# rasmusab/bayes.js

Measured on AMD Instinct MI355X. Metric: posterior draws/sec (= param-updates/sec), higher is better.
Workload: dtype f64

## Files before the change

bayes.js_amd/csrc/amwg_eval.h:

```cpp
#pragma once
#include "amwg_kernel.h"
#include "amwg_user.h"

namespace amwg {

AMWG_HD double ld_by_id(int id, double x, double a, double b, double c) {
  switch (id) {
    case 0: return ld_norm(x, a, b);
    case 1: return ld_unif(x, a, b);
    case 2: return ld_beta(x, a, b);
    case 3: return ld_bern(x, a);
    case 4: return ld_pois(x, a);
    case 5: return ld_cauchy(x, a, b);
    case 6: return ld_laplace(x, a, b);
    case 7: return ld_gamma(x, a, b);
    case 8: return ld_invgamma(x, a, b);
    case 9: return ld_lnorm(x, a, b);
    case 10: return ld_pareto(x, a, b);
    case 11: return ld_t(x, a, b, c);
    case 12: return ld_weibull(x, a, b);
    case 13: return ld_logis(x, a, b);
    case 14: return ld_exp(x, a);
    case 15: return ld_binom(x, a, b);
    case 16: return ld_nbinom(x, a, b);
// ... 61 lines not shown
    case 19: r = quot_plain(x, y); break;
    case 20: r = math1_by_id((int)y, x); break;
    case 21: r = atan2_v8(x, y); break;
    case 22: r = hypot3_v8(x, y, z); break;
    case 23: r = hypot2_v8(x, y); break;
    case 24: r = js_mod(x, y); break;
    case 25: r = (double)js_toint32(x); break;
    case 26: { double lam; r = exp_log_v8(x, lam, exp_log_regs()); } break;
    case 27: { double lam; (void)exp_log_v8(x, lam, exp_log_regs()); r = lam; } break;
    case 28: r = exp_v8_full(x); break;
    case 29: r = log_v8_full(x); break;
    case 30: r = log_v8_full(exp_v8_full(x)); break;
    case 31: { double lam; r = exp_log_v8(x, lam, ExpLogLiterals{}); } break;
    case 32: r = log1p_exp_v8(x); break;
    case 33: r = log1p_exp_v8(x, exp_log_regs()); break;
    case 34: r = log1p_v8(exp_v8_full(x)); break;
    case 35: { bool rare = false; r = log1p_exp_v8_open(rare, x); if (rare) r = log1p_exp_cold(x); } break;
    case 36: r = softplus_bounded(x); break;
    case 37: r = softplus_bounded(x, softplus_regs()); break;
  }
  out[i] = r;
}

}
```

bayes.js_amd/csrc/amwg_kernel.h:

```cpp
#pragma once
#if !defined(__HIPCC_RTC__)
#include <hip/hip_runtime.h>
#endif

#include "amwg_div.h"
#include "amwg_ld.h"
#include "amwg_philox.h"
#include "amwg_types.h"

namespace amwg {

struct LdsLayout {
  uint32_t data, state, pls, cnt, tot, cc, adapt, pl, idx, perm, total, stride, logpls, bc, xw;
};
__host__ __device__ inline LdsLayout lds_layout(size_t data_bytes, int P, int CPB, int max_top, int n_named, bool multi = false) {
  LdsLayout L;
  uint32_t o = 0;
  L.stride = (uint32_t)P | 1u;
  L.data = o;  o += (uint32_t)((data_bytes + 15) & ~(size_t)15);
  L.state = o; o += L.stride * CPB * 8;
  L.pls = o;   o += L.stride * CPB * 8;
  L.cnt = o;   o += L.stride * CPB * 8;
  L.tot = o;   o += (L.stride * CPB * 4 + 15) & ~15u;
  L.cc = o;    o += (uint32_t)P * sizeof(CompConst);
  L.adapt = o; o += ((uint32_t)P + 7) & ~7u;
  L.pl = o;    o += (uint32_t)n_named * 20u;
  o = (o + 15) & ~15u;
  L.idx = o;   o += (max_top > 1) ? (((uint32_t)max_top * CPB * (max_top > kByteTop ? 2u : 1u) + 15) & ~15u) : 0;
  L.perm = o;  o += (n_named > kPackedNamed) ? (((uint32_t)n_named * CPB * 2u + 15) & ~15u) : 0;
  L.logpls = o; o += multi ? L.stride * CPB * 8 : 0;
// ... 213 lines not shown
    b0 = consumed >> 1;
    pos = (uint32_t)(consumed & 1u);
    fill();
  }
  __device__ __forceinline__ uint64_t consumed() const { return 2 * b0 + (uint64_t)pos; }
  __device__ __forceinline__ double next() {
    if constexpr (L == 64) {
      uint32_t p = (uint32_t)__builtin_amdgcn_readfirstlane((int)pos);
      if (p >= 128u) { b0 += 64ull; p = 0u; fill(); }
      const double mine = (p & 1u) ? u1 : u0;
      const int src = (int)(p >> 1);
      const uint32_t hi = (uint32_t)__builtin_amdgcn_readlane((int)(f64_bits(mine) >> 32), src);
      const uint32_t lo = (uint32_t)__builtin_amdgcn_readlane((int)(uint32_t)f64_bits(mine), src);
      pos = p + 1u;
      return bits_f64(((uint64_t)hi << 32) | (uint64_t)lo);
    } else {
      if (pos >= 2u * (uint32_t)L) { b0 += (uint64_t)L; pos = 0u; fill(); }
      double mine = (pos & 1u) ? u1 : u0;
      if constexpr (L > 1) mine = __shfl(mine, base_lane + (int)(pos >> 1), 64);
      ++pos;
      return mine;
    }
  }
};

template <int G>
__device__ __forceinline__ bool chain_true(bool c) {
#if defined(__HIP_DEVICE_COMPILE__)
  if constexpr (G >= 64) return __ballot(c) != 0ull;
#endif
  return c;
}

__device__ inline __attribute__((noinline)) int certified_test_wide(double dA, double eta, double u) {
  const double lo = dA - eta, hi = dA + eta;
  if (hi < -746.0) return -1;
  if (lo >= 0.0) return 1;
  if (!(eta < 0x1p+9) || !(u > 0x1p-60)) return 0;
  if (exp_v8(lo) * (1.0 - 0x1p-50) > u) return 1;
  if (exp_v8(hi) * (1.0 + 0x1p-50) < u) return -1;
  return 0;
}
__device__ __forceinline__ int certified_test(double dA, double eta, double ex, double u) {
  if (eta < 0x1p-7) return (ex * (1.0 - eta) > u && (u > 0.0 || dA > -700.0)) ? 1 : (ex * (1.0 + eta) < u ? -1 : 0);
  return certified_test_wide(dA, eta, u);
}

template <class Rng>
__device__ __forceinline__ double rnorm_js(Rng &rng, double mean, double sd) {
  constexpr int GU = Rng::kLanesPerChain;
  double u, v, q;
  bool again;
  do {
    u = rng.next();
    v = 1.7156 * (rng.next() - 0.5);
    const double x = u - 0.449871;
    const double y = __builtin_fabs(v) + 0.386595;
    q = x * x + y * (0.19600 * y - 0.25472 * x);
    again = false;
    if (chain_true<GU>(q > 0.27597)) again = chain_true<GU>(q > 0.27846) || chain_true<GU>(v * v > -4 * log_v8_cold(u) * u * u);
  } while (again);
  return (v / u) * sd + mean;
}

struct IndexColumn {
  unsigned char *base;
  int CPB;
  bool wide;
  __device__ __forceinline__ int get(int t) const {
    return wide ? (int)reinterpret_cast<const uint16_t *>(base)[t * CPB] : (int)base[t * CPB];
  }
  __device__ __forceinline__ void set(int t, int v) const {
    if (wide) reinterpret_cast<uint16_t *>(base)[t * CPB] = (uint16_t)v; else base[t * CPB] = (uint8_t)v;
  }
};
__device__ __forceinline__ uint32_t perm_get(uint64_t perm, int i) { return (uint32_t)(perm >> (4 * i)) & 0xFu; }
__device__ __forceinline__ uint64_t perm_swap(uint64_t perm, int i, int j) {
  const uint64_t d = ((perm >> (4 * i)) ^ (perm >> (4 * j))) & 0xFull;
  return perm ^ (d << (4 * i)) ^ (d << (4 * j));
}

__device__ __forceinline__ double js_max2(double a, double b) {
  if (a != a || b != b) return __builtin_nan("");
  if (a == b) return (a == 0 && __builtin_signbit(a)) ? b : a;
  return a > b ? a : b;
}

template <class M, int G, bool GL, bool SW = false> struct RngOf { using type = CoopStream<G>; };
template <class M, int G> struct RngOf<M, G, true, false> { using type = typename M::Stream; };
template <class M, int G> struct RngOf<M, G, false, true> { using type = typename M::SweepStream; };
template <class M, class = void> struct DynamicLdsOf { static constexpr bool value = false; };
template <class M> struct DynamicLdsOf<M, void_of<decltype(M::kDynamicLds)>> { static constexpr bool value = M::kDynamicLds; };
template <class M, bool GL> struct DataBytesOf {
  static __device__ __forceinline__ size_t get(const DataRef &d, int lanes, int threads) {
    if constexpr (DynamicLdsOf<M>::value) return M::lds_bytes_of(d, lanes, threads);
    else return M::lds_bytes(d.n_obs, d.G, lanes);
  }
};
template <class M> struct DataBytesOf<M, true> { static __device__ __forceinline__ size_t get(const DataRef &d, int, int threads) { return M::gl_lds_bytes(d.pad, threads / 64); } };

#if defined(__HIP_DEVICE_COMPILE__)
typedef const StepArgs __attribute__((address_space(4))) *cold_args_ptr;
__device__ __forceinline__ cold_args_ptr cold_args() {
  cold_args_ptr p = (cold_args_ptr)__builtin_amdgcn_kernarg_segment_ptr();
  asm volatile("" : "+s"(p));
  return p;
}
#else
typedef const StepArgs *cold_args_ptr;
__device__ inline cold_args_ptr cold_args() { return nullptr; }
#endif

struct SlotPre {
// ... 75 lines not shown
#endif
  return v;
}

__device__ __forceinline__ double lane_value(double v, int src) {
#if defined(__HIP_DEVICE_COMPILE__)
  const uint32_t hi = (uint32_t)__builtin_amdgcn_readlane((int)(f64_bits(v) >> 32), src);
  const uint32_t lo = (uint32_t)__builtin_amdgcn_readlane((int)(uint32_t)f64_bits(v), src);
  return bits_f64(((uint64_t)hi << 32) | (uint64_t)lo);
#else
  return v;
#endif
}

constexpr int kErrReplicasNeedOneWave = 1, kErrLaunchTooLong = 2, kErrMirrorOutOfSync = 4, kErrSweepNeedsOrderInRegisters = 8, kErrNoKernelBody = 16;
__device__ __forceinline__ void device_error(const StepArgs &a, int code) {
#if defined(__HIP_DEVICE_COMPILE__)
  if (threadIdx.x == 0) (void)atomicOr(a.ch.error, code);
#endif
}
template <class M, class = void> struct MirrorCheckOf { static constexpr bool value = false; };
template <class M> struct MirrorCheckOf<M, void_of<decltype(M::kMirrorCheck)>> { static constexpr bool value = M::kMirrorCheck; };

template <class Model, int G, int BT = 256, bool GL = false, bool SW = false, bool CT = false>
__device__ __forceinline__ void step_body(const StepArgs &a, unsigned char *smem) {
  constexpr int kPassU = SW ? (CertNeedsRows<Model>::value ? 2 : 4) : (BT >= 1024 ? 4 : 8);
  const int tid = threadIdx.x, nt = blockDim.x;
  constexpr bool kMulti = G > 64;
  if (!kMulti && a.cpb > 0 && nt != 64) { device_error(a, kErrReplicasNeedOneWave); return; }
  if (a.n_steps > 65535) { device_error(a, kErrLaunchTooLong); return; }
  const int CPB = kMulti ? G / 64 : ((a.cpb > 0 && a.cpb < nt / G) ? a.cpb : nt / G);
  const int c_raw = kMulti ? tid / 64 : tid / G;
  const int c_in = c_raw < CPB ? c_raw : CPB - 1, sub = tid % G;
  const int P = a.pl.P;
  const int n_named = a.pl.n_params;
  const LdsLayout L = lds_layout(DataBytesOf<Model, GL>::get(a.d, G, nt), P, CPB, a.pl.max_top, n_named, kMulti);

  const unsigned char *data_lds = smem + L.data;
  double *Sblk = reinterpret_cast<double *>(smem + L.state);
  CompConst *cc = reinterpret_cast<CompConst *>(smem + L.cc);
  uint8_t *adapt = smem + L.adapt;
  int32_t *pl_base = reinterpret_cast<int32_t *>(smem + L.pl), *pl_len = pl_base + n_named, *pl_top = pl_len + n_named, *pl_multidim = pl_top + n_named, *pl_inner = pl_multidim + n_named;
  const bool wide_idx = a.pl.max_top > kByteTop, wide_perm = n_named > kPackedNamed;
  const IndexColumn idx{smem + L.idx + (wide_idx ? 2 * c_in : c_in), CPB, wide_idx};
  const IndexColumn pcol{smem + L.perm + 2 * c_in, CPB, true};
  double *SDme = reinterpret_cast<double *>(smem + L.pls) + (size_t)c_in * L.stride;
  int2 *CNTme = reinterpret_cast<int2 *>(smem + L.cnt) + (size_t)c_in * L.stride;
// ... 7 lines not shown
  for (int p = tid; p < P; p += nt) { cc[p] = a.cc[p]; adapt[p] = a.is_adapting[p]; }
  for (int i = tid; i < 4 * n_named; i += nt) pl_base[i] = a.pl.tab[i];
  for (int i = tid; i < n_named; i += nt) pl_inner[i] = a.pl.tab[n_named + i] / a.pl.tab[2 * n_named + i];

  const int64_t chain_raw = kMulti ? (int64_t)blockIdx.x : (int64_t)blockIdx.x * CPB + c_in;
  const bool live = chain_raw < a.C;
  const int64_t cl = live ? chain_raw : a.C - 1;
  const bool writer = live && sub == 0;
  const bool counter = sub == 0 && c_raw < CPB;
  const int64_t C = a.C;

  double *Sme = Sblk + (size_t)c_in * L.stride;
  for (int p = 0; p < P; ++p) {
    Sme[p] = a.ch.state[p * C + cl];
    SDme[p] = exp_v8(a.ch.prop_log_scale[p * C + cl]);
    CNTme[p] = make_int2(a.ch.acceptance_count[p * C + cl], a.ch.iterations_since_adaption[p * C + cl]);
    TOTme[p] = 0u;
    if constexpr (kMulti) { LOGPLSme[p] = a.ch.prop_log_scale[p * C + cl]; BCme[p] = a.ch.batch_count[p * C + cl]; }
  }
  const StateView S{Sme};
  uint64_t perm = wide_perm ? 0ull : a.ch.perm[cl];
  if (wide_perm)
    for (int k = 0; k < n_named; ++k) pcol.set(k, (int)a.ch.perm16[(int64_t)k * C + cl]);
  typename RngOf<Model, G, GL, SW>::type rng;
  if constexpr (GL) rng.init(a.seed, a.chain_offset + (uint64_t)cl, a.ch.rng_n[cl], tid, reinterpret_cast<double *>(smem + L.data + Model::gl_lds_bytes(a.d.pad, 0)) + (size_t)(tid >> 6) * 256);
  else if constexpr (SW) rng.init(a.seed, a.chain_offset + (uint64_t)cl, a.ch.rng_n[cl], tid, reinterpret_cast<double *>(smem + L.data + Model::window_offset(a.d, nt / 64)) + (size_t)(tid >> 6) * 256);
  else rng.init(a.seed, a.chain_offset + (uint64_t)cl, a.ch.rng_n[cl], tid);
  double lp_curr = a.ch.lp_curr[cl];
  __syncthreads();
  constexpr bool kCert = CT && CertifiedAt<Model, G>::value && !GL && (SW == CertNeedsRows<Model>::value);
  static_assert(kCert == CT, "a certified kernel is instantiated for a model that has no certified value at this lane count");
  constexpr bool kRefOrder = kCert && G > 1 && RefOrderOf<Model>::value;
  auto expression = [&]() -> double {
    if constexpr (kRefOrder) return Model::template reference_order<G>(cache, S, a.mc, a.d, data_lds, sub);
    else if constexpr (!GL) return log_post<Model, G, kPassU>(S, a, data_lds, sub, xw, cache);
    else return 0.0;
  };
  if constexpr (!GL) { if (a.init_lp) lp_curr = expression(); }
  double lpA = lp_curr, epsA = 0.0;
  bool lp_exact = true;
  if constexpr (kCert) { if (!a.init_lp) { epsA = a.ch.lp_eps[cl]; lp_exact = epsA == 0.0; } }
  (void)lpA; (void)epsA; (void)lp_exact;
#if defined(AMWG_AUDIT)
  constexpr bool kAudit = kCert;
#else
  constexpr bool kAudit = false;
#endif
  [[maybe_unused]] double audE = 0.0, aud_max_v = 0.0, aud_max_d = 0.0;
  [[maybe_unused]] uint32_t aud_n = 0u, aud_bad = 0u;
// ... 268 lines not shown
          p_s = p;
          rng.pos = p;
          if (t_begin < top) p_s = rng.position();
        }
        lp_curr = Model::total(gl, lane64, gl.pm, gl.pt, gl.T);
      }
    }
  } else
  for (int step = 0; step < n_steps; ++step) {
    AMWG_PHASE(15);
    record_draws(step);
    shuffle_named();
    AMWG_PHASE(0);
    int np = 0, e = 0, e_top = 0, e_in = 0;
    double sw_prop = 0.0, sw_u = 0.0;
    int ord_pos = lane64;
    (void)ord_pos;
    int sw_left = 0;
    int sb = 0;
    if constexpr (kSweep) sb = Model::sweep_base(a.d);
    bool sw_pending = false;
    int d_len = 1, d_base = 0, d_multi = 0, d_inner = 1;
    auto next_comp = [&]() -> int {
      if (e == 0) {
        const int p = chain_uniform<G>(wide_perm ? pcol.get(np) : (int)perm_get(perm, np));
        d_len = chain_uniform<G>(pl_len[p]);
        d_base = chain_uniform<G>(pl_base[p]);
        d_multi = chain_uniform<G>(pl_multidim[p]);
        if (d_multi) {
          const int top = chain_uniform<G>(pl_top[p]);
          d_inner = chain_uniform<G>(pl_inner[p]);
          if (ord_in_regs) {
#if defined(__HIP_DEVICE_COMPILE__)
            if constexpr (kSweep) {
              const uint32_t p0 = rng.position();
              rng.ensure_b();
              const double uf = rng.at(lane64 >= 1 && lane64 < top ? p0 + (uint32_t)(top - 1 - lane64) : 0u);
              const int jv = (int)__builtin_floor(uf * (double)(lane64 + 1));
              int posc = lane64, i = top - 1;
              for (; i >= 4; i -= 4) {
                const int j0 = __builtin_amdgcn_readlane(jv, i), j1 = __builtin_amdgcn_readlane(jv, i - 1), j2 = __builtin_amdgcn_readlane(jv, i - 2), j3 = __builtin_amdgcn_readlane(jv, i - 3);
                posc = posc == i ? j0 : (posc == j0 ? i : posc);
                posc = posc == i - 1 ? j1 : (posc == j1 ? i - 1 : posc);
                posc = posc == i - 2 ? j2 : (posc == j2 ? i - 2 : posc);
                posc = posc == i - 3 ? j3 : (posc == j3 ? i - 3 : posc);
              }
              for (; i > 0; --i) {
                const int j = __builtin_amdgcn_readlane(jv, i);
                posc = posc == i ? j : (posc == j ? i : posc);
              }
              rng.pos = p0 + (uint32_t)(top - 1);
              ord_pos = posc;
              ord = __builtin_amdgcn_ds_permute(posc << 2, lane64);
            } else if constexpr (G >= 64) {
              ord = lane64;
              for (int i = top - 1; i > 0; --i) {
                const int j = __builtin_amdgcn_readfirstlane((int)__builtin_floor(rng.next() * (double)(i + 1)));
                const int ti = __builtin_amdgcn_readlane(ord, i), tj = __builtin_amdgcn_readlane(ord, j);
                ord = lane64 == i ? tj : (lane64 == j ? ti : ord);
              }
            }
#endif
          } else {
            for (int t = 0; t < top; ++t) idx.set(t, t);
            for (int i = top - 1; i > 0; --i) {
              const int j = (int)__builtin_floor(rng.next() * (double)(i + 1));
              const int ti = idx.get(i);
              idx.set(i, idx.get(j));
              idx.set(j, ti);
            }
          }
          if constexpr (kSweep) sw_pending = sweep_rt && d_base == Model::sweep_base(a.d) && d_inner == 1 && d_len == chain_uniform<G>(Model::sweep_len(a.d)) && d_len > 1;
        }
      }
      int comp = d_base;
      if (d_multi) {
        int t = 0;
        if (ord_in_regs) {
#if defined(__HIP_DEVICE_COMPILE__)
          if constexpr (G >= 64) t = __builtin_amdgcn_readlane(ord, __builtin_amdgcn_readfirstlane(e_top));
#endif
        } else t = idx.get(e_top);
        comp += t * d_inner + e_in;
        if (++e_in == d_inner) { e_in = 0; ++e_top; }
      }
      if (++e == d_len) { e = 0; e_top = 0; e_in = 0; ++np; }
      return comp;
    };
    auto prefetch = [&](int comp) -> SlotPre {
      SlotPre q;
      q.comp = comp;
      q.cur = Sme[comp];
      q.sd = SDme[comp];
      q.cnt = CNTme[comp];
      q.batch_size = cc[comp].batch_size;
// ... 216 lines not shown
        set_state(comp, 1.0);
        const double one_ld = log_post<Model, G, kPassU>(S, a, data_lds, sub, xw, cache);
        const double mx = js_max2(zero_ld, one_ld);
        const double z = zero_ld - mx, o = one_ld - mx;
        const double zero_prob = exp_v8(z - log_v8(exp_v8(z) + exp_v8(o)));
        double now = 1.0;
        lp_curr = one_ld;
        if (rng.next() < zero_prob) { set_state(comp, 0.0); now = 0.0; lp_curr = zero_ld; }
        if (counter) (void)__hip_atomic_fetch_add(&TOTme[comp], 1u + ((now != old) ? 0x10000u : 0u), __ATOMIC_RELAXED, __HIP_MEMORY_SCOPE_WORKGROUP);
        if (slot + 1 < P_stepped) nx = prefetch(next_comp());
        continue;
      }
      AMWG_PHASE(14);
      const double cur = me.cur;
      const bool in_sweep = kSweep && sw_left > 0;
      double prop;
      if (in_sweep) prop = lane_value(sw_prop, comp - sb);
      else {
        prop = rnorm_js(rng, cur, me.sd);
        if (chain_true<G>(k_type == kTypeInt)) prop = js_round(prop);
      }
      const bool inb = chain_true<G>(!(prop < k_lower || prop > k_upper));
      double u_accept = 0.0;
      if (inb) { set_state(comp, prop); u_accept = in_sweep ? lane_value(sw_u, comp - sb) : rng.next(); }
      if (in_sweep) --sw_left;
      AMWG_PHASE(8);
      if (slot + 1 < P_stepped) nx = prefetch(next_comp());
      AMWG_PHASE(9);
      bool accepted = false;
      bool certified = false;
      [[maybe_unused]] double aud_E_prop = 0.0;
      if constexpr (kCert) {
        if (__ballot(inb) != 0ull) {
          wave_priority(0);
          const typename Model::Approx r = Model::template log_post_approx<G, BT>(cache, S, a.mc, a.d, data_lds, sub);
          wave_priority(kStepperPriority);
          AMWG_PHASE(10);
          if (inb) {
            const double dA = r.value - lpA;
            const double eta = ((r.eps + epsA + __builtin_fabs(dA) * 0x1p-51) * 1.0625 + 0x1p-49) * a.bound_scale;
            const double ex = exp_v8(dA);
            if constexpr (kAudit) { if (a.audit_adversarial) u_accept = audit_adversarial_u(ex, eta, u_accept, step + slot); }
            const int verdict = certified_test(dA, eta, ex, u_accept);
            if constexpr (kAudit) {
              aud_E_prop = expression();
              audit_value(r.value, r.eps, aud_E_prop);
              audit_difference(dA, (r.eps + epsA + __builtin_fabs(dA) * 0x1p-51) * 1.0625, aud_E_prop - audE, verdict, u_accept);
// ... 121 lines not shown
```

bayes.js_amd/csrc/amwg_plan.hip:

```cpp
#include <algorithm>
#include <cmath>
#include <cstdlib>

#include "amwg_host.h"
#include "amwg_kernel.h"
#include "amwg_models.h"

using namespace amwg;

const FamilyRow *family_of(int model) {
  static const FamilyRow rows[4] = {amwg_family_row<0>(), amwg_family_row<1>(), amwg_family_row<2>(), amwg_family_row<3>()};
  return model >= AMWG_MODEL_NORMAL && model <= AMWG_MODEL_POIS_GLM ? &rows[model - 1] : nullptr;
}

int gl_layout(const double *y, const int32_t *g, int N, int Gn, GlLayoutHost *out) {
  if (Gn < 1 || Gn > 64) return amwg_fail(AMWG_EINVAL, "group_local: 1 to 64 groups (a chain runs on one wavefront, a lane serves one group), got %d", Gn);
  std::vector<int> n(Gn, 0), L(Gn, 1), first(Gn, 0);
  for (int i = 0; i < N; ++i) {
    if (g[i] < 0 || g[i] >= Gn) return amwg_fail(AMWG_EINVAL, "group_local: g[%d] = %d outside 0..%d", i, g[i], Gn - 1);
    n[g[i]]++;
  }
  int total = Gn;
  for (;;) {
    int best = 0;
// ... 72 lines not shown
  const bool cert = decide_certified && ((s->model == AMWG_MODEL_NORMAL && G == 1) || (s->model == AMWG_MODEL_POIS_GLM && G == 16) || rows) &&
                    family_of(s->model)->certified(G, bt).plain != nullptr;
  p.variant = rows ? (cert ? Variant::HierSweepCert : Variant::HierSweep) : (cert ? Variant::StepCert : Variant::Step);
  p.pad = rows ? HierNormalModel::row_pitch(s->d.n_obs) : ((cert && s->model == AMWG_MODEL_NORMAL && bt <= 512 && !o.sufficient_statistics) ? 1 : 0);
  return p;
}

static bool row_layout(const amwg_sampler *s, const LaunchPlan &p) {
  return p.variant == Variant::HierSweep || p.variant == Variant::HierSweepCert || (s->user && p.pad > 0);
}

static uint32_t lds_of_size(const amwg_sampler *s, const LaunchPlan &p, int cpb, int n_obs) {
  const int G = p.lanes, bt = p.block;
  size_t data = 0;
  switch (p.variant) {
    case Variant::GroupLocal: data = HierGlModel::gl_lds_bytes(p.pad, bt / 64); break;
    case Variant::HierSweep: case Variant::HierSweepCert: data = HierNormalModel::rows_lds_bytes(p.pad, bt / 64, s->d.G); break;
    case Variant::Step: case Variant::StepCert:
      data = (s->model == AMWG_MODEL_NORMAL && G == 1) ? (p.pad ? NormalModel::one_lane_tile_bytes(n_obs) : 0) : family_of(s->model)->lds_bytes(n_obs, s->d.G, G);
      break;
    default:
      data = p.pad ? HierNormalModel::rows_lds_bytes(p.pad, bt / 64, s->user_rows_groups) : (size_t)(G == 1 ? s->user_lds_one_lane : s->user_lds);
  }
  return G > 64 ? lds_layout(data, s->P, G / 64, s->pl.max_top, s->n_params, true).total : lds_layout(data, s->P, cpb ? cpb : bt / G, s->pl.max_top, s->n_params).total;
}

static uint32_t lds_of(const amwg_sampler *s, const LaunchPlan &p, int cpb = 0) {
  if (s->n_datasets <= 1) return lds_of_size(s, p, cpb, s->d.n_obs);
  uint32_t most = 0;
  int last = -1;
  for (int n : s->ds_n_obs) {
    if (n == last) continue;
    most = std::max(most, lds_of_size(s, p, cpb, n));
    last = n;
  }
  return most;
}

static int priced_n_obs(const amwg_sampler *s) {
  if (s->n_datasets <= 1) return s->d.n_obs;
  int64_t sum = 0;
  for (int n : s->ds_n_obs) sum += n;
  return (int)((sum + s->n_datasets - 1) / s->n_datasets);
}
static int log2_of(int lanes) { int lg = 0; for (int g = lanes; g > 1; g >>= 1) ++lg; return lg; }
static double model_work(const amwg_sampler *s, int G) {
  const LaunchPlan q = variant_for(s, G, 256, (size_t)160 * 1024);
// ... 228 lines not shown
```

bayes.js_amd/csrc/amwg_rtc.hip:

```cpp
#include <hip/hiprtc.h>
#include <fcntl.h>
#include <sys/stat.h>
#include <unistd.h>

#include <cstdio>
#include <cstdlib>
#include <cstring>
#include <map>
#include <mutex>

#include "amwg_host.h"

extern "C" {
extern const char amwg_hdr_stdint[], amwg_hdr_types[], amwg_hdr_math[], amwg_hdr_div[], amwg_hdr_ld[], amwg_hdr_philox[],
    amwg_hdr_kernel[], amwg_hdr_user[], amwg_hdr_twoval[], amwg_hdr_kval[], amwg_hdr_trig[], amwg_hdr_pass[], amwg_hdr_rows[], amwg_hdr_window[], amwg_hdr_gtail[],
    amwg_hdr_user_kernels[], amwg_hdr_user_dataset[];
}

static std::string user_program(const char *source, int lanes, int block) {
  return "#include \"amwg_kernel.h\"\n#include \"amwg_user.h\"\n#define AMWG_USER_LANES " + std::to_string(lanes) + "\n#define AMWG_USER_BLOCK " + std::to_string(block) + "\n" +
         source + "\n#include \"amwg_user_kernels.h\"\n";
}

namespace {
struct CacheKey { uint64_t h1, h2, h3; uint64_t len; };
CacheKey hash_key(const std::vector<std::string> &parts) {
  CacheKey k{0xcbf29ce484222325ull, 0x84222325cbf29ce4ull, 0x9e3779b97f4a7c15ull, 0};
  for (const std::string &p : parts) {
    for (unsigned char c : p) {
      k.h1 = (k.h1 ^ c) * 0x100000001b3ull;
      k.h2 = (k.h2 + c + (k.h2 << 6) + (k.h2 >> 2)) * 0xff51afd7ed558ccdull;
      k.h3 = ((k.h3 << 5) | (k.h3 >> 59)) ^ (c * 0xc4ceb9fe1a85ec53ull);
    }
    k.h1 = (k.h1 ^ 0xff) * 0x100000001b3ull;
    k.len += p.size() + 1;
  }
  return k;
}
// ... 38 lines not shown
void cache_write(const std::string &dir, const std::string &file, const CacheKey &k, const std::vector<char> &code) {
  make_dirs(dir);
  if (!cache_dir_trusted(dir)) return;
  const std::string tmp = file + ".tmp." + std::to_string((long)getpid());
  const int fd = open(tmp.c_str(), O_WRONLY | O_CREAT | O_EXCL | O_NOFOLLOW | O_CLOEXEC, 0600);
  if (fd < 0) return;
  FILE *f = fdopen(fd, "wb");
  if (!f) { close(fd); (void)remove(tmp.c_str()); return; }
  const uint64_t hdr[4] = {k.h2, k.h3, k.len, payload_sum(code)}, n = code.size();
  const bool ok = fwrite(kCacheMagic, 1, 8, f) == 8 && fwrite(hdr, 8, 4, f) == 4 && fwrite(&n, 8, 1, f) == 1 && fwrite(code.data(), 1, code.size(), f) == code.size();
  if (fclose(f) != 0 || !ok || rename(tmp.c_str(), file.c_str()) != 0) (void)remove(tmp.c_str());
}
std::atomic<int> g_cache_hits{0}, g_cache_misses{0};
}

static void dump_code_object(const std::vector<char> &code) {
  if (const char *dump = getenv("AMWG_DUMP_CODE_OBJECT")) {
    if (FILE *f = fopen(dump, "wb")) { fwrite(code.data(), 1, code.size(), f); fclose(f); }
  }
}

static int compile_user(const char *source, int lanes, int block, const char *arch, std::vector<char> *code, bool datasets, bool use_cache = true) {
  static const char *names[] = {"amwg_stdint.h", "amwg_types.h", "amwg_math.h", "amwg_div.h", "amwg_ld.h", "amwg_philox.h", "amwg_kernel.h", "amwg_user.h",
                                "amwg_twoval.h", "amwg_kval.h", "amwg_trig.h", "amwg_pass.h", "amwg_rows.h", "amwg_window.h", "amwg_gtail.h", "amwg_user_kernels.h", "amwg_user_dataset.h"};
  const char *texts[] = {amwg_hdr_stdint, amwg_hdr_types, amwg_hdr_math, amwg_hdr_div, amwg_hdr_ld, amwg_hdr_philox, amwg_hdr_kernel, amwg_hdr_user,
                         amwg_hdr_twoval, amwg_hdr_kval, amwg_hdr_trig, amwg_hdr_pass, amwg_hdr_rows, amwg_hdr_window, amwg_hdr_gtail, amwg_hdr_user_kernels, amwg_hdr_user_dataset};
  constexpr int kHeaders = (int)(sizeof(texts) / sizeof(texts[0]));
  const std::string prog_src = user_program(source, lanes, block);
#if defined(AMWG_AUDIT)
  const char *const kOpts[] = {"-O3", "-std=c++17", "-ffp-contract=off", "-fno-fast-math", "-Wno-unused-value", "-DAMWG_AUDIT=1"};
#elif defined(AMWG_X_PHASES)
  const char *const kOpts[] = {"-O3", "-std=c++17", "-ffp-contract=off", "-fno-fast-math", "-Wno-unused-value", "-DAMWG_X_PHASES=1"};
#else
  const char *const kOpts[] = {"-O3", "-std=c++17", "-ffp-contract=off", "-fno-fast-math", "-Wno-unused-value", "-falign-loops=64"};
#endif
  static const char *const kDatasetsOpt = "-DAMWG_USER_DATASETS=1";
  std::string dir = cache_dir(), file;
  CacheKey key{};
  if (!dir.empty()) {
    int rt_major = 0, rt_minor = 0;
    (void)hiprtcVersion(&rt_major, &rt_minor);
    std::vector<std::string> parts = {prog_src, arch, "hiprtc " + std::to_string(rt_major) + "." + std::to_string(rt_minor)};
    for (const char *o : kOpts) parts.push_back(o);
    if (datasets) parts.push_back(kDatasetsOpt);
    for (const char *t : texts) parts.push_back(t);
    key = hash_key(parts);
    char name[64];
    snprintf(name, sizeof name, "/%016llx%016llx.hsaco", (unsigned long long)key.h1, (unsigned long long)key.h2);
    file = dir + name;
// ... 100 lines not shown
```

bayes.js_amd/csrc/amwg_rtc_headers.c:

```c
#define AMWG_TEXT(sym, file)                                                        \
  __asm__(".section .rodata\n.global " #sym "\n.type " #sym ", @object\n" #sym ":\n" \
          ".incbin \"" file "\"\n.byte 0\n.size " #sym ", .-" #sym "\n.text\n")
AMWG_TEXT(amwg_hdr_stdint, "amwg_stdint.h");
AMWG_TEXT(amwg_hdr_types, "amwg_types.h");
AMWG_TEXT(amwg_hdr_math, "amwg_math.h");
AMWG_TEXT(amwg_hdr_div, "amwg_div.h");
AMWG_TEXT(amwg_hdr_ld, "amwg_ld.h");
AMWG_TEXT(amwg_hdr_philox, "amwg_philox.h");
AMWG_TEXT(amwg_hdr_kernel, "amwg_kernel.h");
AMWG_TEXT(amwg_hdr_user, "amwg_user.h");
AMWG_TEXT(amwg_hdr_twoval, "amwg_twoval.h");
AMWG_TEXT(amwg_hdr_kval, "amwg_kval.h");
AMWG_TEXT(amwg_hdr_trig, "amwg_trig.h");
AMWG_TEXT(amwg_hdr_pass, "amwg_pass.h");
AMWG_TEXT(amwg_hdr_rows, "amwg_rows.h");
AMWG_TEXT(amwg_hdr_window, "amwg_window.h");
AMWG_TEXT(amwg_hdr_gtail, "amwg_gtail.h");
AMWG_TEXT(amwg_hdr_user_kernels, "amwg_user_kernels.h");
AMWG_TEXT(amwg_hdr_user_dataset, "amwg_user_dataset.h");
```

bayes.js_amd/csrc/amwg_selftest.hip:

```cpp
#include "../../include/amwg_selftest.h"
#include "amwg_dataset_quantiles.h"
#include "amwg_autocov.h"
#include "amwg_covariance.h"
#include "amwg_fold.h"
#include "amwg_histogram.h"
#include "amwg_hpd.h"
#include "amwg_eval.h"
#include "amwg_host.h"
#include "amwg_kernel.h"
#include "amwg_models.h"

using namespace amwg;
__global__ void two_valued_check_kernel(const uint32_t *tab, int N, int64_t m, const double *acc0, const double *l1, const double *l0,
                                        double *out_ff, double *out_seq) {
  const int64_t j = (int64_t)blockIdx.x * blockDim.x + threadIdx.x;
  if (j >= m) return;
  const size_t W = BetaBernModel::words(N);
  BitData B{tab, tab + W, tab + 2 * W, tab + 3 * W, tab + 4 * W, tab + 5 * W, N};
  out_ff[j] = two_valued_sum(acc0[j], l1[j], l0[j], B);
  double acc = acc0[j];
  for (int i = 0; i < N; ++i) acc = acc + (((tab[i >> 5] >> (i & 31)) & 1u) ? l1[j] : l0[j]);
  out_seq[j] = acc;
}

// ... 50 lines not shown
int amwg_ld_device(int32_t device, int64_t n, const double *records, double *out) {
  if (!records || !out || n < 0) return amwg_fail(AMWG_EINVAL, "amwg_ld_device: bad argument");
  TRYB(use_device(device));
  DevBuf dr, dout;
  HIP_TRY(dr.alloc((size_t)n * 40));
  HIP_TRY(dout.alloc((size_t)n * 8));
  HIP_TRY(hipMemcpy(dr.p, records, (size_t)n * 40, hipMemcpyHostToDevice));
  if (n) hipLaunchKernelGGL(amwg_ld_eval_kernel, dim3((unsigned)((n + 255) / 256)), dim3(256), 0, 0, n, dr.as<double>(), dout.as<double>());
  HIP_TRY(hipGetLastError());
  HIP_TRY(hipMemcpy(out, dout.p, (size_t)n * 8, hipMemcpyDeviceToHost));
  return AMWG_OK;
}

int amwg_device_eval(int32_t device, int32_t op, int64_t n, const double *a, const double *b, const double *c, double *out) {
  if (!a || !out || n < 0) return amwg_fail(AMWG_EINVAL, "amwg_device_eval: bad argument");
  TRYB(use_device(device));
  DevBuf da, db, dc, dout;
  const size_t bytes = (size_t)n * 8;
  HIP_TRY(da.alloc(bytes));
  HIP_TRY(dout.alloc(bytes));
  HIP_TRY(hipMemcpy(da.p, a, bytes, hipMemcpyHostToDevice));
  if (b) { HIP_TRY(db.alloc(bytes)); HIP_TRY(hipMemcpy(db.p, b, bytes, hipMemcpyHostToDevice)); }
  if (c) { HIP_TRY(dc.alloc(bytes)); HIP_TRY(hipMemcpy(dc.p, c, bytes, hipMemcpyHostToDevice)); }
  if (n) hipLaunchKernelGGL(amwg_eval_kernel, dim3((unsigned)((n + 255) / 256)), dim3(256), 0, 0, op, n, da.as<double>(), db.as<double>(), dc.as<double>(), dout.as<double>());
  HIP_TRY(hipGetLastError());
  HIP_TRY(hipMemcpy(out, dout.p, bytes, hipMemcpyDeviceToHost));
  return AMWG_OK;
}

int amwg_dataset_quantiles_check(int32_t device, const double *draws, int64_t rows, int32_t PR, int64_t C, int32_t D, const double *probs, int32_t n_probs, double *out) {
  if (!draws || !probs || !out) return amwg_fail(AMWG_EINVAL, "amwg_dataset_quantiles_check: null argument");
  TRYB(amwg_dataset_quantiles_shape("amwg_dataset_quantiles_check", rows, PR, C, D, n_probs));
  if (rows > INT64_MAX / 8 / PR / C) return amwg_fail(AMWG_EINVAL, "amwg_dataset_quantiles_check: array too large");
  TRYB(use_device(device));
  const size_t bytes = (size_t)rows * (size_t)PR * (size_t)C * 8;
  DevBuf dd;
  HIP_TRY(dd.alloc(bytes));
  HIP_TRY(hipMemcpy(dd.p, draws, bytes, hipMemcpyHostToDevice));
  return amwg_dataset_quantiles_launch("amwg_dataset_quantiles_check", dd.as<double>(), rows, PR, C, D, probs, n_probs, out, nullptr);
}

int amwg_hpd_check(int32_t device, const double *draws, int64_t rows, int32_t PR, int64_t C, int32_t D, const double *probs, int32_t n_probs, double *out) {
  if (!draws || !probs || !out) return amwg_fail(AMWG_EINVAL, "amwg_hpd_check: null argument");
  TRYB(amwg_hpd_shape("amwg_hpd_check", rows, PR, C, D, n_probs));
  if (rows > INT64_MAX / 8 / PR / C) return amwg_fail(AMWG_EINVAL, "amwg_hpd_check: array too large");
  TRYB(use_device(device));
// ... 126 lines not shown
```

bayes.js_amd/csrc/amwg_user_dataset.h:

```cpp
#pragma once
#include "amwg_kernel.h"

namespace amwg {

struct UserDatasetArgs {
  int32_t blocks_per_dataset, n_datasets;
  int32_t row_stride, n_arrays;
  const void *const *table;
};

__device__ __forceinline__ void user_dataset_view(StepArgs &v, const UserDatasetArgs &ds) {
#if defined(__HIP_DEVICE_COMPILE__)
  const int64_t d = (int64_t)__builtin_amdgcn_readfirstlane((int)(blockIdx.x / (uint32_t)ds.blocks_per_dataset));
#else
  const int64_t d = 0;
#endif
  const void *const *row = ds.table + d * (int64_t)ds.row_stride;
#pragma unroll
  for (int j = 0; j < kInlineUserArrays; ++j) v.d.arr[j] = row[j];
  v.d.arr_ext = row + kInlineUserArrays;
}

}

#if defined(AMWG_USER_LANES) && defined(AMWG_USER_BLOCK)
extern "C" __global__ void __launch_bounds__(AMWG_USER_BLOCK) amwg_user_step_ds(const amwg::StepArgs a, const amwg::UserDatasetArgs ds) {
  extern __shared__ __attribute__((aligned(16))) unsigned char smem[];
  amwg::StepArgs v = a;
  amwg::user_dataset_view(v, ds);
  amwg::step_body<amwg::UserModel, AMWG_USER_LANES>(v, smem);
}

extern "C" __global__ void __launch_bounds__(AMWG_USER_BLOCK) amwg_user_step_cert_ds(const amwg::StepArgs a, const amwg::UserDatasetArgs ds) {
  extern __shared__ __attribute__((aligned(16))) unsigned char smem[];
  if constexpr (amwg::CertifiedAt<amwg::UserModel, AMWG_USER_LANES>::value && !amwg::CertNeedsRows<amwg::UserModel>::value) {
    amwg::StepArgs v = a;
    amwg::user_dataset_view(v, ds);
    amwg::step_body<amwg::UserModel, AMWG_USER_LANES, (AMWG_USER_BLOCK <= 256 ? 256 : 1024), false, false, true>(v, smem);
  } else amwg::device_error(a, amwg::kErrNoKernelBody);
}
#endif
```

bayes.js_amd/csrc/amwg_user_kernels.h:

```cpp
#if !defined(AMWG_USER_LANES) || !defined(AMWG_USER_BLOCK)
#error "amwg_user_kernels.h: define AMWG_USER_LANES and AMWG_USER_BLOCK first"
#endif

extern "C" __global__ void __launch_bounds__(AMWG_USER_BLOCK) amwg_user_step(const amwg::StepArgs a) {
  extern __shared__ __attribute__((aligned(16))) unsigned char smem[];
  amwg::step_body<amwg::UserModel, AMWG_USER_LANES>(a, smem);
}

extern "C" __global__ void __launch_bounds__(AMWG_USER_BLOCK) amwg_user_sweep(const amwg::StepArgs a) {
  extern __shared__ __attribute__((aligned(16))) unsigned char smem[];
  if constexpr (amwg::LaneReuseOf<amwg::UserModel>::value && AMWG_USER_LANES == 64 && AMWG_USER_BLOCK <= 512) amwg::step_body<amwg::UserModel, 64, 512, false, true>(a, smem);
  else amwg::device_error(a, amwg::kErrNoKernelBody);
}

extern "C" __global__ void __launch_bounds__(AMWG_USER_BLOCK) amwg_user_sweep_cert(const amwg::StepArgs a) {
  extern __shared__ __attribute__((aligned(16))) unsigned char smem[];
  if constexpr (amwg::LaneReuseOf<amwg::UserModel>::value && amwg::CertifiedAt<amwg::UserModel, 64>::value && amwg::CertNeedsRows<amwg::UserModel>::value && AMWG_USER_LANES == 64 &&
                AMWG_USER_BLOCK <= 512)
    amwg::step_body<amwg::UserModel, 64, 512, false, true, true>(a, smem);
  else amwg::device_error(a, amwg::kErrNoKernelBody);
}

extern "C" __global__ void __launch_bounds__(AMWG_USER_BLOCK) amwg_user_step_cert(const amwg::StepArgs a) {
  extern __shared__ __attribute__((aligned(16))) unsigned char smem[];
  if constexpr (amwg::CertifiedAt<amwg::UserModel, AMWG_USER_LANES>::value && !amwg::CertNeedsRows<amwg::UserModel>::value)
    amwg::step_body<amwg::UserModel, AMWG_USER_LANES, (AMWG_USER_BLOCK <= 256 ? 256 : 1024), false, false, true>(a, smem);
  else amwg::device_error(a, amwg::kErrNoKernelBody);
}

#if defined(AMWG_USER_DATASETS)
#include "amwg_user_dataset.h"
#endif
```

bayes.js_amd/csrc/amwg_window.h:

```cpp
#pragma once
#if !defined(__HIPCC_RTC__)
#include <hip/hip_runtime.h>
#endif

#include "amwg_math.h"
#include "amwg_philox.h"

namespace amwg {

struct WindowStream {
  static constexpr int kLanesPerChain = 64;
  uint32_t k0, k1, c2, c3;
  uint64_t b0;
  uint32_t pos;
  double a0, a1, b0v, b1v;
  uint64_t EA, OA, EB, OB;
  bool b_valid;
  double *win;
  int lane;
  static __device__ __attribute__((noinline)) Philox4 block(uint64_t b, uint32_t c2, uint32_t c3, uint32_t k0, uint32_t k1) {
    return philox4x32_10((uint32_t)b, (uint32_t)(b >> 32), c2, c3, k0, k1);
  }
  static __device__ __forceinline__ bool pair_ok(double u, double v_raw) {
#if defined(AMWG_X_GLCUT) && AMWG_X_GLCUT == 7
// ... 61 lines not shown
    b0 += 64ull;
    a0 = b0v; a1 = b1v;
    EA = EB; OA = OB;
    store_a();
    b_valid = false;
  }
  __device__ __forceinline__ uint64_t consumed() const { return 2 * b0 + (uint64_t)pos; }
  __device__ __forceinline__ uint32_t position() {
#if defined(__HIP_DEVICE_COMPILE__)
    uint32_t p = (uint32_t)__builtin_amdgcn_readfirstlane((int)pos);
#else
    uint32_t p = pos;
#endif
    while (p >= 128u) { shift(); p -= 128u; }
    pos = p;
    return p;
  }
  __device__ __forceinline__ double next() {
    const uint32_t p = position();
    const double mine = (p & 1u) ? a1 : a0;
    pos = p + 1u;
    return from_lane(mine, (int)(p >> 1));
  }
  __device__ __forceinline__ double at(uint32_t q) const { return win[q & 255u]; }
};

}
```

Before: 1.472 billion.

## Add lockstep Philox stream with LDS FIFO for one-lane-per-chain kernels

Introduces LockstepStream, which serves one-lane-per-chain (G==1) chains. Each lane keeps a small LDS ring of prefetched Philox uniforms and refills only when some lane in the wavefront runs out, so the whole wavefront shares one refill. The normal rejection sampler, the Fisher-Yates shuffle and the accept draw are rewritten as ballot-driven lockstep loops using next_if, so divergent lanes stop issuing separate Philox calls. This costs extra LDS per block and adds wavefront-wide loops that run until the slowest lane finishes.

```diff
diff --git a/bayes.js_amd/csrc/amwg_eval.h b/bayes.js_amd/csrc/amwg_eval.h
--- a/bayes.js_amd/csrc/amwg_eval.h
+++ b/bayes.js_amd/csrc/amwg_eval.h
@@ -107,4 +107,21 @@
   out[i] = r;
 }
 
+constexpr int kEvalStreamOp = 38;
+template <int SLOTS>
+__global__ void __launch_bounds__(64) amwg_stream1_eval_kernel(int64_t n, const double *a, const double *b, const double *c, double *out) {
+  __shared__ __attribute__((aligned(16))) unsigned char fifo[SLOTS * 1024];
+  const int lane = (int)threadIdx.x, T = (int)(n / 64), live = (int)b[2];
+  if (live < 1 || live > 64 || T < 1) return;
+  const int col = lane < live ? lane : live - 1;
+  LockstepStream<SLOTS> s;
+  s.init((uint64_t)b[0], (uint64_t)b[1] + (uint64_t)col, (uint64_t)c[col], lane, fifo);
+  for (int t = 0; t + 1 < T; ++t) {
+    const bool take = a[(int64_t)t * 64 + col] != 0.0;
+    const double u = s.next_if(take);
+    out[(int64_t)t * 64 + lane] = lane < live ? (take ? u : -1.0) : -2.0;
+  }
+  out[(int64_t)(T - 1) * 64 + lane] = lane < live ? (double)s.consumed() : -2.0;
 }
+
+}
diff --git a/bayes.js_amd/csrc/amwg_kernel.h b/bayes.js_amd/csrc/amwg_kernel.h
--- a/bayes.js_amd/csrc/amwg_kernel.h
+++ b/bayes.js_amd/csrc/amwg_kernel.h
@@ -6,6 +6,7 @@
 #include "amwg_div.h"
 #include "amwg_ld.h"
 #include "amwg_philox.h"
+#include "amwg_stream1.h"
 #include "amwg_types.h"
 
 namespace amwg {
@@ -265,6 +266,7 @@
       return mine;
     }
   }
+  __device__ __forceinline__ double next_if(bool c) { return c ? next() : 0.0; }
 };
 
 template <int G>
@@ -294,6 +296,23 @@
   constexpr int GU = Rng::kLanesPerChain;
   double u, v, q;
   bool again;
+  if constexpr (LockstepOf<Rng>::value) {
+    u = 0.0; v = 0.0;
+    again = true;
+    do {
+      const double un = rng.next_if(again), vn = rng.next_if(again);
+      if (again) {
+        u = un;
+        v = 1.7156 * (vn - 0.5);
+        const double x = u - 0.449871;
+        const double y = __builtin_fabs(v) + 0.386595;
+        q = x * x + y * (0.19600 * y - 0.25472 * x);
+        again = false;
+        if (q > 0.27597) again = q > 0.27846 || v * v > -4 * log_v8_cold(u) * u * u;
+      }
+    } while (__ballot(again) != 0ull);
+    return (v / u) * sd + mean;
+  }
   do {
     u = rng.next();
     v = 1.7156 * (rng.next() - 0.5);
@@ -329,9 +348,10 @@
   return a > b ? a : b;
 }
 
-template <class M, int G, bool GL, bool SW = false> struct RngOf { using type = CoopStream<G>; };
-template <class M, int G> struct RngOf<M, G, true, false> { using type = typename M::Stream; };
-template <class M, int G> struct RngOf<M, G, false, true> { using type = typename M::SweepStream; };
+template <class M, int G, bool GL, bool SW = false, int NT = 256> struct RngOf { using type = CoopStream<G>; };
+template <class M, int G, int NT> struct RngOf<M, G, true, false, NT> { using type = typename M::Stream; };
+template <class M, int G, int NT> struct RngOf<M, G, false, true, NT> { using type = typename M::SweepStream; };
+template <class M, int NT> struct RngOf<M, 1, false, false, NT> { using type = LockstepStream<stream1_slots(NT)>; };
 template <class M, class = void> struct DynamicLdsOf { static constexpr bool value = false; };
 template <class M> struct DynamicLdsOf<M, void_of<decltype(M::kDynamicLds)>> { static constexpr bool value = M::kDynamicLds; };
 template <class M, bool GL> struct DataBytesOf {
@@ -453,7 +473,7 @@
 template <class M, class = void> struct MirrorCheckOf { static constexpr bool value = false; };
 template <class M> struct MirrorCheckOf<M, void_of<decltype(M::kMirrorCheck)>> { static constexpr bool value = M::kMirrorCheck; };
 
-template <class Model, int G, int BT = 256, bool GL = false, bool SW = false, bool CT = false>
+template <class Model, int G, int BT = 256, bool GL = false, bool SW = false, bool CT = false, int NT = BT>
 __device__ __forceinline__ void step_body(const StepArgs &a, unsigned char *smem) {
   constexpr int kPassU = SW ? (CertNeedsRows<Model>::value ? 2 : 4) : (BT >= 1024 ? 4 : 8);
   const int tid = threadIdx.x, nt = blockDim.x;
@@ -507,9 +527,11 @@
   uint64_t perm = wide_perm ? 0ull : a.ch.perm[cl];
   if (wide_perm)
     for (int k = 0; k < n_named; ++k) pcol.set(k, (int)a.ch.perm16[(int64_t)k * C + cl]);
-  typename RngOf<Model, G, GL, SW>::type rng;
+  typename RngOf<Model, G, GL, SW, NT>::type rng;
+  constexpr bool kLockRng = LockstepOf<typename RngOf<Model, G, GL, SW, NT>::type>::value;
   if constexpr (GL) rng.init(a.seed, a.chain_offset + (uint64_t)cl, a.ch.rng_n[cl], tid, reinterpret_cast<double *>(smem + L.data + Model::gl_lds_bytes(a.d.pad, 0)) + (size_t)(tid >> 6) * 256);
   else if constexpr (SW) rng.init(a.seed, a.chain_offset + (uint64_t)cl, a.ch.rng_n[cl], tid, reinterpret_cast<double *>(smem + L.data + Model::window_offset(a.d, nt / 64)) + (size_t)(tid >> 6) * 256);
+  else if constexpr (kLockRng) rng.init(a.seed, a.chain_offset + (uint64_t)cl, a.ch.rng_n[cl], tid, smem + L.total);
   else rng.init(a.seed, a.chain_offset + (uint64_t)cl, a.ch.rng_n[cl], tid);
   double lp_curr = a.ch.lp_curr[cl];
   __syncthreads();
@@ -824,6 +846,7 @@
     bool sw_pending = false;
     int d_len = 1, d_base = 0, d_multi = 0, d_inner = 1;
     auto next_comp = [&]() -> int {
+      [[maybe_unused]] int fy_i = 0;
       if (e == 0) {
         const int p = chain_uniform<G>(wide_perm ? pcol.get(np) : (int)perm_get(perm, np));
         d_len = chain_uniform<G>(pl_len[p]);
@@ -865,6 +888,8 @@
 #endif
           } else {
             for (int t = 0; t < top; ++t) idx.set(t, t);
+            if constexpr (kLockRng) fy_i = top - 1;
+            else
             for (int i = top - 1; i > 0; --i) {
               const int j = (int)__builtin_floor(rng.next() * (double)(i + 1));
               const int ti = idx.get(i);
@@ -873,6 +898,19 @@
             }
           }
           if constexpr (kSweep) sw_pending = sweep_rt && d_base == Model::sweep_base(a.d) && d_inner == 1 && d_len == chain_uniform<G>(Model::sweep_len(a.d)) && d_len > 1;
+        }
+      }
+      if constexpr (kLockRng) {
+        while (__ballot(fy_i > 0) != 0ull) {
+          const bool go = fy_i > 0;
+          const double uf = rng.next_if(go);
+          if (go) {
+            const int j = (int)__builtin_floor(uf * (double)(fy_i + 1));
+            const int ti = idx.get(fy_i);
+            idx.set(fy_i, idx.get(j));
+            idx.set(j, ti);
+            --fy_i;
+          }
         }
       }
       int comp = d_base;
@@ -1135,7 +1173,12 @@
       }
       const bool inb = chain_true<G>(!(prop < k_lower || prop > k_upper));
       double u_accept = 0.0;
-      if (inb) { set_state(comp, prop); u_accept = in_sweep ? lane_value(sw_u, comp - sb) : rng.next(); }
+      if constexpr (kLockRng) {
+        if (inb) set_state(comp, prop);
+        u_accept = rng.next_if(inb);
+      } else {
+        if (inb) { set_state(comp, prop); u_accept = in_sweep ? lane_value(sw_u, comp - sb) : rng.next(); }
+      }
       if (in_sweep) --sw_left;
       AMWG_PHASE(8);
       if (slot + 1 < P_stepped) nx = prefetch(next_comp());
diff --git a/bayes.js_amd/csrc/amwg_plan.hip b/bayes.js_amd/csrc/amwg_plan.hip
--- a/bayes.js_amd/csrc/amwg_plan.hip
+++ b/bayes.js_amd/csrc/amwg_plan.hip
@@ -118,7 +118,8 @@
     default:
       data = p.pad ? HierNormalModel::rows_lds_bytes(p.pad, bt / 64, s->user_rows_groups) : (size_t)(G == 1 ? s->user_lds_one_lane : s->user_lds);
   }
-  return G > 64 ? lds_layout(data, s->P, G / 64, s->pl.max_top, s->n_params, true).total : lds_layout(data, s->P, cpb ? cpb : bt / G, s->pl.max_top, s->n_params).total;
+  if (G > 64) return lds_layout(data, s->P, G / 64, s->pl.max_top, s->n_params, true).total;
+  return lds_layout(data, s->P, cpb ? cpb : bt / G, s->pl.max_top, s->n_params).total + (G == 1 ? stream1_lds_bytes(bt) : 0u);
 }
 
 static uint32_t lds_of(const amwg_sampler *s, const LaunchPlan &p, int cpb = 0) {
diff --git a/bayes.js_amd/csrc/amwg_rtc.hip b/bayes.js_amd/csrc/amwg_rtc.hip
--- a/bayes.js_amd/csrc/amwg_rtc.hip
+++ b/bayes.js_amd/csrc/amwg_rtc.hip
@@ -13,7 +13,7 @@
 
 extern "C" {
 extern const char amwg_hdr_stdint[], amwg_hdr_types[], amwg_hdr_math[], amwg_hdr_div[], amwg_hdr_ld[], amwg_hdr_philox[],
-    amwg_hdr_kernel[], amwg_hdr_user[], amwg_hdr_twoval[], amwg_hdr_kval[], amwg_hdr_trig[], amwg_hdr_pass[], amwg_hdr_rows[], amwg_hdr_window[], amwg_hdr_gtail[],
+    amwg_hdr_kernel[], amwg_hdr_user[], amwg_hdr_twoval[], amwg_hdr_kval[], amwg_hdr_trig[], amwg_hdr_pass[], amwg_hdr_rows[], amwg_hdr_window[], amwg_hdr_stream1[], amwg_hdr_gtail[],
     amwg_hdr_user_kernels[], amwg_hdr_user_dataset[];
 }
 
@@ -98,9 +98,9 @@
 
 static int compile_user(const char *source, int lanes, int block, const char *arch, std::vector<char> *code, bool datasets, bool use_cache = true) {
   static const char *names[] = {"amwg_stdint.h", "amwg_types.h", "amwg_math.h", "amwg_div.h", "amwg_ld.h", "amwg_philox.h", "amwg_kernel.h", "amwg_user.h",
-                                "amwg_twoval.h", "amwg_kval.h", "amwg_trig.h", "amwg_pass.h", "amwg_rows.h", "amwg_window.h", "amwg_gtail.h", "amwg_user_kernels.h", "amwg_user_dataset.h"};
+                                "amwg_twoval.h", "amwg_kval.h", "amwg_trig.h", "amwg_pass.h", "amwg_rows.h", "amwg_window.h", "amwg_stream1.h", "amwg_gtail.h", "amwg_user_kernels.h", "amwg_user_dataset.h"};
   const char *texts[] = {amwg_hdr_stdint, amwg_hdr_types, amwg_hdr_math, amwg_hdr_div, amwg_hdr_ld, amwg_hdr_philox, amwg_hdr_kernel, amwg_hdr_user,
-                         amwg_hdr_twoval, amwg_hdr_kval, amwg_hdr_trig, amwg_hdr_pass, amwg_hdr_rows, amwg_hdr_window, amwg_hdr_gtail, amwg_hdr_user_kernels, amwg_hdr_user_dataset};
+                         amwg_hdr_twoval, amwg_hdr_kval, amwg_hdr_trig, amwg_hdr_pass, amwg_hdr_rows, amwg_hdr_window, amwg_hdr_stream1, amwg_hdr_gtail, amwg_hdr_user_kernels, amwg_hdr_user_dataset};
   constexpr int kHeaders = (int)(sizeof(texts) / sizeof(texts[0]));
   const std::string prog_src = user_program(source, lanes, block);
 #if defined(AMWG_AUDIT)
diff --git a/bayes.js_amd/csrc/amwg_rtc_headers.c b/bayes.js_amd/csrc/amwg_rtc_headers.c
--- a/bayes.js_amd/csrc/amwg_rtc_headers.c
+++ b/bayes.js_amd/csrc/amwg_rtc_headers.c
@@ -15,6 +15,7 @@
 AMWG_TEXT(amwg_hdr_pass, "amwg_pass.h");
 AMWG_TEXT(amwg_hdr_rows, "amwg_rows.h");
 AMWG_TEXT(amwg_hdr_window, "amwg_window.h");
+AMWG_TEXT(amwg_hdr_stream1, "amwg_stream1.h");
 AMWG_TEXT(amwg_hdr_gtail, "amwg_gtail.h");
 AMWG_TEXT(amwg_hdr_user_kernels, "amwg_user_kernels.h");
 AMWG_TEXT(amwg_hdr_user_dataset, "amwg_user_dataset.h");
diff --git a/bayes.js_amd/csrc/amwg_selftest.hip b/bayes.js_amd/csrc/amwg_selftest.hip
--- a/bayes.js_amd/csrc/amwg_selftest.hip
+++ b/bayes.js_amd/csrc/amwg_selftest.hip
@@ -96,6 +96,13 @@
   HIP_TRY(hipMemcpy(da.p, a, bytes, hipMemcpyHostToDevice));
   if (b) { HIP_TRY(db.alloc(bytes)); HIP_TRY(hipMemcpy(db.p, b, bytes, hipMemcpyHostToDevice)); }
   if (c) { HIP_TRY(dc.alloc(bytes)); HIP_TRY(hipMemcpy(dc.p, c, bytes, hipMemcpyHostToDevice)); }
+  if (op == kEvalStreamOp) {
+    if (!b || !c || n < 128 || n % 64 != 0) return amwg_fail(AMWG_EINVAL, "amwg_device_eval: op %d takes three arrays of 64 T entries, T >= 2", (int)op);
+    HIP_TRY(hipMemset(dout.p, 0, bytes));
+    if (!(b[3] >= 64 && b[3] <= 1024)) return amwg_fail(AMWG_EINVAL, "amwg_device_eval: op %d: b[3] is a workgroup size, 64 .. 1024", (int)op);
+    if (stream1_slots((int)b[3]) == 4) hipLaunchKernelGGL(amwg_stream1_eval_kernel<4>, dim3(1), dim3(64), 0, 0, n, da.as<double>(), db.as<double>(), dc.as<double>(), dout.as<double>());
+    else hipLaunchKernelGGL(amwg_stream1_eval_kernel<2>, dim3(1), dim3(64), 0, 0, n, da.as<double>(), db.as<double>(), dc.as<double>(), dout.as<double>());
+  } else
   if (n) hipLaunchKernelGGL(amwg_eval_kernel, dim3((unsigned)((n + 255) / 256)), dim3(256), 0, 0, op, n, da.as<double>(), db.as<double>(), dc.as<double>(), dout.as<double>());
   HIP_TRY(hipGetLastError());
   HIP_TRY(hipMemcpy(out, dout.p, bytes, hipMemcpyDeviceToHost));
diff --git a/bayes.js_amd/csrc/amwg_stream1.h b/bayes.js_amd/csrc/amwg_stream1.h
--- /dev/null
+++ b/bayes.js_amd/csrc/amwg_stream1.h
@@ -0,0 +1,78 @@
+#pragma once
+#if !defined(__HIPCC_RTC__)
+#include <hip/hip_runtime.h>
+#endif
+
+#include "amwg_math.h"
+#include "amwg_philox.h"
+
+namespace amwg {
+
+__host__ __device__ constexpr int stream1_slots(int threads) { return threads <= 256 ? 4 : 2; }
+__host__ __device__ constexpr uint32_t stream1_lds_bytes(int threads) { return (uint32_t)((threads + 63) / 64) * (uint32_t)stream1_slots(threads) * 1024u; }
+
+template <int SLOTS>
+struct LockstepStream {
+  static_assert(SLOTS >= 1 && (SLOTS & (SLOTS - 1)) == 0, "a block's slot is its index modulo SLOTS");
+  static constexpr int kLanesPerChain = 1;
+  static constexpr bool kLockstep = true;
+#if defined(__HIP_DEVICE_COMPILE__)
+  typedef double __attribute__((address_space(3))) *lds_f64;
+#else
+  typedef double *lds_f64;
+#endif
+  uint32_t k0, k1, c2, c3;
+  uint64_t n;
+  uint32_t avail;
+  double nxt;
+  uint32_t q;
+  static constexpr uint32_t slots = (uint32_t)SLOTS;
+  static __device__ __attribute__((noinline)) Philox4 block(uint64_t b, uint32_t c2, uint32_t c3, uint32_t k0, uint32_t k1) {
+    return philox4x32_10((uint32_t)b, (uint32_t)(b >> 32), c2, c3, k0, k1);
+  }
+  __device__ __forceinline__ lds_f64 at(uint32_t m) const { return (lds_f64)(uintptr_t)(q + ((m & (2u * slots - 1u)) << 9)); }
+  __device__ __forceinline__ void refill() {
+    const uint64_t b = (n + (uint64_t)avail) >> 1;
+    const Philox4 w = block(b, c2, c3, k0, k1);
+    const double f0 = u53(w.w0, w.w1), f1 = u53(w.w2, w.w3);
+    if (avail + ((uint32_t)n & 1u) < 2u * slots) {
+      const lds_f64 p = at(2u * (uint32_t)b);
+      p[0] = f0; p[64] = f1;
+      if (avail == 0u) nxt = f0;
+      avail += 2u;
+    }
+  }
+  __device__ __forceinline__ void init(uint64_t seed, uint64_t chain, uint64_t consumed, int tid, unsigned char *lds) {
+    k0 = (uint32_t)seed; k1 = (uint32_t)(seed >> 32);
+    c2 = (uint32_t)chain; c3 = (uint32_t)(chain >> 32);
+#if defined(__HIP_DEVICE_COMPILE__)
+    q = (uint32_t)(uintptr_t)(__attribute__((address_space(3))) unsigned char *)lds + (uint32_t)(tid >> 6) * (slots << 10) + (uint32_t)(tid & 63) * 8u;
+#else
+    q = 0;
+#endif
+    n = consumed;
+    const Philox4 w = block(consumed >> 1, c2, c3, k0, k1);
+    const double f0 = u53(w.w0, w.w1), f1 = u53(w.w2, w.w3);
+    const lds_f64 p = at(2u * (uint32_t)(consumed >> 1));
+    p[0] = f0; p[64] = f1;
+    nxt = (consumed & 1u) ? f1 : f0;
+    avail = 2u - (uint32_t)(consumed & 1u);
+  }
+  __device__ __forceinline__ uint64_t consumed() const { return n; }
+  __device__ __forceinline__ double next_if(bool take) {
+    if (__ballot(take && avail == 0u) != 0ull) refill();
+    const double r = nxt;
+    if (take) {
+      n += 1ull;
+      avail -= 1u;
+      if (avail != 0u) nxt = *at((uint32_t)n);
+    }
+    return r;
+  }
+  __device__ __forceinline__ double next() { return next_if(true); }
+};
+
+template <class R, class = void> struct LockstepOf { static constexpr bool value = false; };
+template <class R> struct LockstepOf<R, decltype((void)R::kLockstep)> { static constexpr bool value = R::kLockstep; };
+
+}
diff --git a/bayes.js_amd/csrc/amwg_user_dataset.h b/bayes.js_amd/csrc/amwg_user_dataset.h
--- a/bayes.js_amd/csrc/amwg_user_dataset.h
+++ b/bayes.js_amd/csrc/amwg_user_dataset.h
@@ -28,7 +28,7 @@
   extern __shared__ __attribute__((aligned(16))) unsigned char smem[];
   amwg::StepArgs v = a;
   amwg::user_dataset_view(v, ds);
-  amwg::step_body<amwg::UserModel, AMWG_USER_LANES>(v, smem);
+  amwg::step_body<amwg::UserModel, AMWG_USER_LANES, 256, false, false, false, AMWG_USER_BLOCK>(v, smem);
 }
 
 extern "C" __global__ void __launch_bounds__(AMWG_USER_BLOCK) amwg_user_step_cert_ds(const amwg::StepArgs a, const amwg::UserDatasetArgs ds) {
@@ -36,7 +36,7 @@
   if constexpr (amwg::CertifiedAt<amwg::UserModel, AMWG_USER_LANES>::value && !amwg::CertNeedsRows<amwg::UserModel>::value) {
     amwg::StepArgs v = a;
     amwg::user_dataset_view(v, ds);
-    amwg::step_body<amwg::UserModel, AMWG_USER_LANES, (AMWG_USER_BLOCK <= 256 ? 256 : 1024), false, false, true>(v, smem);
+    amwg::step_body<amwg::UserModel, AMWG_USER_LANES, (AMWG_USER_BLOCK <= 256 ? 256 : 1024), false, false, true, AMWG_USER_BLOCK>(v, smem);
   } else amwg::device_error(a, amwg::kErrNoKernelBody);
 }
 #endif
diff --git a/bayes.js_amd/csrc/amwg_user_kernels.h b/bayes.js_amd/csrc/amwg_user_kernels.h
--- a/bayes.js_amd/csrc/amwg_user_kernels.h
+++ b/bayes.js_amd/csrc/amwg_user_kernels.h
@@ -4,7 +4,7 @@
 
 extern "C" __global__ void __launch_bounds__(AMWG_USER_BLOCK) amwg_user_step(const amwg::StepArgs a) {
   extern __shared__ __attribute__((aligned(16))) unsigned char smem[];
-  amwg::step_body<amwg::UserModel, AMWG_USER_LANES>(a, smem);
+  amwg::step_body<amwg::UserModel, AMWG_USER_LANES, 256, false, false, false, AMWG_USER_BLOCK>(a, smem);
 }
 
 extern "C" __global__ void __launch_bounds__(AMWG_USER_BLOCK) amwg_user_sweep(const amwg::StepArgs a) {
@@ -24,7 +24,7 @@
 extern "C" __global__ void __launch_bounds__(AMWG_USER_BLOCK) amwg_user_step_cert(const amwg::StepArgs a) {
   extern __shared__ __attribute__((aligned(16))) unsigned char smem[];
   if constexpr (amwg::CertifiedAt<amwg::UserModel, AMWG_USER_LANES>::value && !amwg::CertNeedsRows<amwg::UserModel>::value)
-    amwg::step_body<amwg::UserModel, AMWG_USER_LANES, (AMWG_USER_BLOCK <= 256 ? 256 : 1024), false, false, true>(a, smem);
+    amwg::step_body<amwg::UserModel, AMWG_USER_LANES, (AMWG_USER_BLOCK <= 256 ? 256 : 1024), false, false, true, AMWG_USER_BLOCK>(a, smem);
   else amwg::device_error(a, amwg::kErrNoKernelBody);
 }
 
diff --git a/bayes.js_amd/csrc/amwg_window.h b/bayes.js_amd/csrc/amwg_window.h
--- a/bayes.js_amd/csrc/amwg_window.h
+++ b/bayes.js_amd/csrc/amwg_window.h
@@ -107,6 +107,7 @@
     pos = p + 1u;
     return from_lane(mine, (int)(p >> 1));
   }
+  __device__ __forceinline__ double next_if(bool c) { return c ? next() : 0.0; }
   __device__ __forceinline__ double at(uint32_t q) const { return win[q & 255u]; }
 };
 
```

After: 1.482 billion, median of 6. No clear change (+0.6%).
